# openGemini/openGemini

Measured on AMD Instinct MI355X. Metric: points aggregated/sec, higher is better.
Workload: dtype f64; 1 GPU; 100k series x 1k pts float64 Gorilla, mean/min/max/count GROUP BY time(1m), single TSSP file (mode=walk, 100000x1000); window=1m, series_per_gpu=100000, parallelism=shard-per-gpu dp1

## Files before the change

opengemini_amd/csrc/gemx_engine.hip:

```cpp
#include <hip/hip_runtime.h>
#include <stdint.h>
#include <stdio.h>
#include <string.h>
#include <stdlib.h>
#include <math.h>
#include <vector>
#include <map>
#include <tuple>
#include <type_traits>
#include <string>
#include <algorithm>
#include <chrono>

#include "../../include/gemx.h"

#define UVNAN 0x7FF8000000000001ULL
#define INFLUX_MIN_TIME (INT64_MIN + 2)
#define INFLUX_MAX_TIME (INT64_MAX - 1)


__device__ __forceinline__ uint32_t d_u32be(const uint8_t *p) {
  return ((uint32_t)p[0] << 24) | ((uint32_t)p[1] << 16) | ((uint32_t)p[2] << 8) |
         p[3];
}
// ... 23 lines not shown
  return b;
}
__device__ __forceinline__ int64_t d_zigzag_dec(uint64_t u) {
  return (int64_t)((u >> 1) ^ (uint64_t)((int64_t)((u & 1) << 63) >> 63));
}
__device__ __forceinline__ int d_uvarint(const uint8_t *p, int64_t len, uint64_t *out) {
  uint64_t v = 0;
  int s = 0;
  for (int i = 0; i < len && i < 10; i++) {
    uint8_t b = p[i];
    if (b < 0x80) {
      *out = v | ((uint64_t)b << s);
      return i + 1;
    }
    v |= (uint64_t)(b & 0x7f) << s;
    s += 7;
  }
  return 0;
}

__device__ __host__ __forceinline__ int64_t win_floordiv(int64_t a, int64_t b) {
  int64_t q = a / b;
  if ((a % b) != 0 && ((a < 0) != (b < 0))) q--;
  return q;
}
__device__ __host__ __forceinline__ int64_t win_ordinal(int64_t t, int64_t interval,
                                                        int64_t offset) {
  return win_floordiv(t - offset, interval);
}
__device__ __host__ __forceinline__ int64_t win_start_of(int64_t ord, int64_t interval,
                                                         int64_t offset) {
  int64_t s = ord * interval + offset;
  return s;
}


struct BitR {
  const uint8_t *b;
  int64_t len, pos;
  uint64_t hi, lo;
  int have;

  uint64_t pw;
  int pwbits;

  __device__ __forceinline__ void preload() {
    if (len - pos >= 8) {
      pw = d_u64be(b + pos);
      pos += 8;
      pwbits = 64;
    } else if (pos < len) {
      int rem = (int)(len - pos);
      uint64_t w = 0;
      for (int i = 0; i < rem; i++) w = (w << 8) | b[pos + i];
      pw = w << ((8 - rem) * 8);
      pos = len;
      pwbits = rem * 8;
    } else {
      pw = 0;
      pwbits = 0;
    }
  }

  __device__ __forceinline__ void fill_one() {
    unsigned __int128 ins = ((unsigned __int128)pw << 64) >> have;
    hi |= (uint64_t)(ins >> 64);
    lo |= (uint64_t)ins;
    have += pwbits;
    preload();
  }

  __device__ __forceinline__ void fill() {
    while (pwbits && have + pwbits <= 128) {
      if (have == 0) {
        hi = pw;
        lo = 0;
      } else if (have < 64) {
        hi |= pw >> have;
        lo |= pw << (64 - have);
      } else if (have == 64) {
        lo |= pw;
      } else {
        lo |= pw >> (have - 64);
      }
      have += pwbits;
      preload();
    }
  }

  __device__ __forceinline__ void init(const uint8_t *p, int64_t n) {
    b = p;
    len = n;
    pos = 0;
    hi = lo = 0;
    have = 0;
    pwbits = 0;
    preload();
    fill();
  }

  __device__ __forceinline__ int read(int n, uint64_t *out) {
    if (have < n) {
      fill();
      if (have < n) return -1;
    }
    uint64_t v = (n == 64) ? hi : (hi >> (64 - n));
    hi = (n == 64) ? lo : ((hi << n) | (lo >> (64 - n)));
    lo = (n == 64) ? 0 : (lo << n);
    have -= n;
    if (have <= 64) fill();
    *out = v;
    return 0;
  }

  __device__ __forceinline__ void consume(int n) {
    unsigned __int128 w = (((unsigned __int128)hi << 64) | lo) << n;
    hi = (uint64_t)(w >> 64);
    lo = (uint64_t)w;
    have -= n;
    if (have <= 64) fill_one();
  }
};

struct GorDesc {
  uint64_t first_val;
  uint64_t arena_base;
  int64_t t0, dt;
};

struct GorA {
  const uint64_t *p;
  uint64_t w0, w1, w2, w3;
  uint64_t M;
  uint32_t np;

  __device__ __forceinline__ void init(const uint64_t *arena, uint64_t base,
                                       uint32_t bp = 0) {
    p = arena + base;
    w0 = p[0 * 64];
    w1 = p[1 * 64];
    w2 = p[2 * 64];
    w3 = p[3 * 64];
    M = p[4 * 64];
    p += 4 * 64;
    np = bp;
  }
  __device__ __forceinline__ void advance(uint32_t nb) {
    np = nb;
    p += (uint64_t)(nb >> 6) << 6;
  }
  template <bool MASKED = true>
  __device__ __forceinline__ void settle() {
    const bool c = np >= 64;
    w0 = c ? w1 : w0;
    w1 = c ? w2 : w1;
    w2 = c ? w3 : w2;
    w3 = c ? M : w3;
    if (!MASKED || c) M = *p;
    if (__builtin_expect(__any(np >= 128), 0)) {
      const bool c2 = np >= 128;
      const uint64_t x = *(p - 64);
      asm volatile("" : "+v"(w1), "+v"(w2), "+v"(w3));
      w0 = c2 ? w1 : w0;
      w1 = c2 ? w2 : w1;
      w2 = c2 ? w3 : w2;
      w3 = c2 ? x : w3;
    }
    np &= 63;
  }
  __device__ __forceinline__ uint32_t word_idx(const uint64_t *base) const {
    return (uint32_t)((p - base) >> 6) - 4;
  }
  static __device__ __forceinline__ uint64_t fun(uint64_t a, uint64_t b,
                                                 uint32_t bp) {
    return (a << bp) | ((b >> (63 - bp)) >> 1);
  }
};

#define GEMX_ARENA_PAD_WORDS ((uint64_t)(2 * 4097 + 32) * 64)


struct FloatIter {
  int kind;
  const uint8_t *raw;
  int64_t raw_n, raw_i;
  double same_v;
  int64_t same_n, same_i;
  const uint8_t *rle_p;
  int64_t rle_len, rle_pos;
  int64_t run_left;
  double run_v;
  BitR br;
  GorA ga;
  int use_arena;
  uint64_t g_val;
  uint8_t g_trail, g_mean;
  int g_first, g_done;

  __device__ int init_gor_arena(const uint64_t *arena, const GorDesc *g) {
    kind = 3;
    use_arena = 1;
    g_val = g->first_val;
    g_done = (g_val == UVNAN);
    g_first = 1;
    g_trail = 0;
    g_mean = 64;
    ga.init(arena, g->arena_base);
    return 0;
  }

  __device__ int init(const uint8_t *enc, int64_t len) {
    if (len < 1) return -1;
    kind = enc[0] >> 4;
    const uint8_t *in = enc + 1;
    int64_t inlen = len - 1;
    switch (kind) {
    case 0:
      raw = in;
      raw_n = inlen / 8;
      raw_i = 0;
      return 0;
    case 4:
      if (inlen < 2) return -1;
      same_n = ((int64_t)in[0] << 8) | in[1];
      same_v = (inlen == 2) ? 0.0 : d_f64le(in + 2);
      same_i = 0;
      return 0;
    case 5:
      rle_p = in;
      rle_len = inlen;
      rle_pos = 0;
      run_left = 0;
      return 0;
    case 3:
      use_arena = 0;
      if (inlen < 9) { g_done = 1; g_first = 0; return 0; }
      g_val = d_u64be(in + 1);
      g_done = (g_val == UVNAN);
      g_first = 1;
      g_trail = 0;
      g_mean = 64;
      br.init(in + 9, inlen - 9);
      return 0;
    default:
      return -2;
    }
  }

  __device__ int next(double *out) {
    switch (kind) {
    case 0:
      if (raw_i >= raw_n) return -1;
      *out = d_f64le(raw + raw_i * 8);
      raw_i++;
      return 0;
    case 4:
      if (same_i >= same_n) return -1;
      *out = same_v;
      same_i++;
      return 0;
    case 5:
      while (run_left == 0) {
        if (rle_len - rle_pos < 2) return -1;
        uint16_t m = (uint16_t)(((uint16_t)rle_p[rle_pos] << 8) | rle_p[rle_pos + 1]);
        if (m >> 15) {
          run_left = m & 0x7FFF;
          run_v = 0.0;
          rle_pos += 2;
        } else {
          if (rle_len - rle_pos < 10) return -1;
          run_left = m;
          run_v = d_f64le(rle_p + rle_pos + 2);
          rle_pos += 10;
        }
      }
      *out = run_v;
      run_left--;
      return 0;
    case 3: {
      if (g_first) {
        if (g_done) return -1;
        g_first = 0;
        uint64_t u = g_val;
        memcpy(out, &u, 8);
        return 0;
      }
      if (g_done) return -1;
      if (use_arena) {
        uint64_t A = GorA::fun(ga.w0, ga.w1, ga.np);
        uint32_t p13 = (uint32_t)(A >> 51);
        uint32_t ctrl1 = p13 >> 12;
        uint32_t neww = ctrl1 & ((p13 >> 11) & 1);
        uint32_t mr = p13 & 0x3F;
        g_mean = neww ? (uint8_t)(mr ? mr : 64u) : g_mean;
        g_trail =
            neww ? (uint8_t)(mr ? (64u - ((p13 >> 6) & 0x1F) - mr) : 0u)
                 : g_trail;
        uint32_t hdr = 1 + ctrl1 + (neww ? 11u : 0u);
        uint64_t Cc = GorA::fun(ga.w1, ga.w2, ga.np);
        uint64_t B = (A << hdr) | (Cc >> (64 - hdr));
        uint64_t sbv = (g_mean == 64) ? B : (B >> (64 - g_mean));
        g_val ^= ctrl1 ? (sbv << (g_trail & 63)) : 0;
        if (g_val == UVNAN) {
          g_done = 1;
          return -1;
        }
        ga.advance(ga.np + hdr + (ctrl1 ? (uint32_t)g_mean : 0));
        ga.settle<false>();
        uint64_t u = g_val;
        memcpy(out, &u, 8);
        return 0;
// ... 1972 lines not shown
        at[op] = p.t[op];
        continue;
      }
      switch (op) {
      case 0: av[op].i += p.v[op].i; break;
      case 1:
        if (COLTYPE == GEMX_TYPE_FLOAT) av[op].f += p.v[op].f;
        else av[op].i += p.v[op].i;
        break;
      case 2: {
        int repl = (COLTYPE == GEMX_TYPE_FLOAT) ? (p.v[op].f < av[op].f)
                                                : (p.v[op].i < av[op].i);
        if (repl) { av[op] = p.v[op]; at[op] = p.t[op]; }
        break;
      }
      case 3: {
        int repl = (COLTYPE == GEMX_TYPE_FLOAT) ? (p.v[op].f > av[op].f)
                                                : (p.v[op].i > av[op].i);
        if (repl) { av[op] = p.v[op]; at[op] = p.t[op]; }
        break;
      }
      case 4: break;
      case 5: av[op] = p.v[op]; at[op] = p.t[op]; break;
      }
    }
  }
  if (!any) return 0;
  out->count = active[0] ? av[0].i : 0;
  out->count_time = active[0] ? at[0] : nt[0];
  out->sum = av[1];
  out->sum_time = active[1] ? at[1] : nt[1];
  out->sum_isnil = !active[1];
  out->minv = av[2];
  out->min_time = active[2] ? at[2] : nt[2];
  out->min_isnil = !active[2];
  out->maxv = av[3];
  out->max_time = active[3] ? at[3] : nt[3];
  out->max_isnil = !active[3];
  out->firstv = av[4];
  out->first_time = active[4] ? at[4] : nt[4];
  out->first_isnil = !active[4];
  out->lastv = av[5];
  out->last_time = active[5] ? at[5] : nt[5];
  out->last_isnil = !active[5];
  if (!active[1]) out->sum.i = 0;
  if (!active[2]) out->minv.i = 0;
  if (!active[3]) out->maxv.i = 0;
  if (!active[4]) out->firstv.i = 0;
  if (!active[5]) out->lastv.i = 0;
  return 1;
}

template <int COLTYPE>
__global__ void __launch_bounds__(256) k_merge(
    const SeriesQ *__restrict__ series, uint32_t nseries,
    const SegQ *__restrict__ segq, const Partial *__restrict__ partials,
    gemx_agg_row *__restrict__ rows, uint64_t total_rows, int64_t interval,
    int64_t offset, int64_t q_start, DevErr *__restrict__ err) {
  uint64_t gid = blockIdx.x * (uint64_t)blockDim.x + threadIdx.x;
  for (uint64_t r = gid; r < total_rows; r += gridDim.x * (uint64_t)blockDim.x) {
    uint32_t lo = 0, hi = nseries - 1;
    while (lo < hi) {
      uint32_t mid = (lo + hi + 1) >> 1;
      if (series[mid].out_base <= r) lo = mid;
      else hi = mid - 1;
    }
    const SeriesQ s = series[lo];
    int64_t w = s.w_min + (int64_t)(r - s.out_base);
    gemx_agg_row out;
    memset(&out, 0, sizeof(out));
    out.sid = s.sid;
    out.win_start = interval ? win_start_of(w, interval, offset) : q_start;
    if (!merge_series_window<COLTYPE>(s, segq, partials, w, &out)) {
      out.count = -1;
      __hip_atomic_fetch_add(&err->gaps, 1ull, __ATOMIC_RELAXED,
                            __HIP_MEMORY_SCOPE_SYSTEM);
    }
    rows[r] = out;
  }
}


template <int COLTYPE>
__device__ __forceinline__ void gacc_row(GAcc *a, const gemx_agg_row *r,
                                         uint32_t src) {
  a->used = 1;
  a->count += r->count;
  if (!r->sum_isnil) {
    if (!(a->active & 2)) {
      a->sum = r->sum;
      a->active |= 2;
    } else if (COLTYPE == GEMX_TYPE_FLOAT)
      a->sum.f += r->sum.f;
    else
      a->sum.i += r->sum.i;
  }
  if (!r->min_isnil) {
    int take = !(a->active & 4);
    if (!take) {
      take = (COLTYPE == GEMX_TYPE_FLOAT)
                 ? (r->minv.f < a->minv.f ||
                    (r->minv.f == a->minv.f && r->min_time < a->min_t))
                 : (r->minv.i < a->minv.i ||
                    (r->minv.i == a->minv.i && r->min_time < a->min_t));
    }
    if (take) {
      a->minv = r->minv;
      a->min_t = r->min_time;
      a->min_src = src;
      a->active |= 4;
    }
  }
  if (!r->max_isnil) {
    int take = !(a->active & 8);
    if (!take) {
      take = (COLTYPE == GEMX_TYPE_FLOAT)
                 ? (r->maxv.f > a->maxv.f ||
                    (r->maxv.f == a->maxv.f && r->max_time < a->max_t))
                 : (r->maxv.i > a->maxv.i ||
                    (r->maxv.i == a->maxv.i && r->max_time < a->max_t));
    }
    if (take) {
      a->maxv = r->maxv;
      a->max_t = r->max_time;
      a->max_src = src;
      a->active |= 8;
    }
  }
  if (!r->first_isnil) {
    if (!(a->active & 16) || r->first_time < a->first_t) {
      a->firstv = r->firstv;
      a->first_t = r->first_time;
      a->first_src = src;
      a->active |= 16;
    }
  }
  if (!r->last_isnil) {
    if (!(a->active & 32) || r->last_time > a->last_t) {
      a->lastv = r->lastv;
      a->last_t = r->last_time;
      a->last_src = src;
      a->active |= 32;
    }
  }
}

template <int COLTYPE>
__device__ __forceinline__ void gacc_merge(GAcc *l, const GAcc *r) {
  if (!r->used) return;
  l->used = 1;
  l->count += r->count;
  if (r->active & 2) {
    if (!(l->active & 2)) {
      l->sum = r->sum;
      l->active |= 2;
    } else if (COLTYPE == GEMX_TYPE_FLOAT)
      l->sum.f += r->sum.f;
    else
      l->sum.i += r->sum.i;
  }
  if (r->active & 4) {
    int take = !(l->active & 4);
    if (!take)
      take = (COLTYPE == GEMX_TYPE_FLOAT)
                 ? (r->minv.f < l->minv.f ||
                    (r->minv.f == l->minv.f &&
                     (r->min_t < l->min_t ||
                      (r->min_t == l->min_t && r->min_src < l->min_src))))
                 : (r->minv.i < l->minv.i ||
                    (r->minv.i == l->minv.i &&
                     (r->min_t < l->min_t ||
                      (r->min_t == l->min_t && r->min_src < l->min_src))));
    if (take) {
      l->minv = r->minv;
      l->min_t = r->min_t;
      l->min_src = r->min_src;
      l->active |= 4;
    }
  }
  if (r->active & 8) {
    int take = !(l->active & 8);
    if (!take)
      take = (COLTYPE == GEMX_TYPE_FLOAT)
                 ? (r->maxv.f > l->maxv.f ||
                    (r->maxv.f == l->maxv.f &&
                     (r->max_t < l->max_t ||
                      (r->max_t == l->max_t && r->max_src < l->max_src))))
                 : (r->maxv.i > l->maxv.i ||
                    (r->maxv.i == l->maxv.i &&
                     (r->max_t < l->max_t ||
                      (r->max_t == l->max_t && r->max_src < l->max_src))));
    if (take) {
      l->maxv = r->maxv;
      l->max_t = r->max_t;
      l->max_src = r->max_src;
      l->active |= 8;
    }
  }
  if (r->active & 16) {
    if (!(l->active & 16) || r->first_t < l->first_t ||
        (r->first_t == l->first_t && r->first_src < l->first_src)) {
      l->firstv = r->firstv;
      l->first_t = r->first_t;
      l->first_src = r->first_src;
      l->active |= 16;
    }
  }
  if (r->active & 32) {
    if (!(l->active & 32) || r->last_t > l->last_t ||
        (r->last_t == l->last_t && r->last_src < l->last_src)) {
      l->lastv = r->lastv;
      l->last_t = r->last_t;
      l->last_src = r->last_src;
      l->active |= 32;
    }
  }
}

template <int COLTYPE, bool FOLD = false>
__global__ void __launch_bounds__(256) k_group_p1(
    const SeriesQ *__restrict__ series, uint32_t nseries,
    const SegQ *__restrict__ segq, const Partial *__restrict__ partials,
    GAcc *__restrict__ gtmp, int64_t W0, uint32_t n_gwins, uint32_t split,
    uint32_t per_chunk, const uint32_t *__restrict__ sel = nullptr,
    const uint8_t *__restrict__ seg_folded = nullptr) {
  __shared__ GAcc sh[256];
  for (uint32_t bb = blockIdx.x; bb < n_gwins * split; bb += gridDim.x) {
    uint32_t wb = bb / split, c = bb % split;
    int64_t w = W0 + (int64_t)wb;
    uint32_t g0 = c * per_chunk;
    uint32_t g1 = g0 + per_chunk;
    if (g1 > nseries) g1 = nseries;
    GAcc a;
    memset(&a, 0, sizeof(a));
    for (uint32_t gi = g0 + threadIdx.x; gi < g1; gi += blockDim.x) {
      const uint32_t g = FOLD ? sel[gi] : gi;
      const SeriesQ s = series[g];
      int64_t local = w - s.w_min;
      if (local < 0 || local >= (int64_t)s.n_wins) continue;
      gemx_agg_row r;
      memset(&r, 0, sizeof(r));
      if (!merge_series_window<COLTYPE, FOLD>(s, segq, partials, w, &r,
                                              seg_folded))
        continue;
      gacc_row<COLTYPE>(&a, &r, g);
    }
    sh[threadIdx.x] = a;
    __syncthreads();
    for (int s2 = 128; s2 > 0; s2 >>= 1) {
      if (threadIdx.x < (uint32_t)s2)
        gacc_merge<COLTYPE>(&sh[threadIdx.x], &sh[threadIdx.x + s2]);
      __syncthreads();
    }
    if (threadIdx.x == 0) gtmp[bb] = sh[0];
    __syncthreads();
  }
}

template <int COLTYPE>
__global__ void __launch_bounds__(256) k_group_p2(
    const GAcc *__restrict__ gtmp, uint32_t split, gemx_agg_row *__restrict__ out,
    int64_t W0, uint32_t n_gwins, int64_t interval, int64_t offset,
    int64_t q_start, int keep_empty, DevErr *__restrict__ err,
    const GAcc *__restrict__ fold = nullptr, uint32_t n_fold = 0) {
  __shared__ GAcc sh[256];
  for (uint32_t wb = blockIdx.x; wb < n_gwins; wb += gridDim.x) {
    int64_t w = W0 + (int64_t)wb;
    GAcc a;
    memset(&a, 0, sizeof(a));
    for (uint32_t c = threadIdx.x; c < split; c += blockDim.x)
      gacc_merge<COLTYPE>(&a, &gtmp[wb * split + c]);
    for (uint32_t c = threadIdx.x; c < n_fold; c += blockDim.x)
      gacc_merge<COLTYPE>(&a, &fold[(uint64_t)wb * n_fold + c]);
    sh[threadIdx.x] = a;
    __syncthreads();
    for (int s = 128; s > 0; s >>= 1) {
      if (threadIdx.x < (uint32_t)s)
        gacc_merge<COLTYPE>(&sh[threadIdx.x], &sh[threadIdx.x + s]);
      __syncthreads();
    }
    if (threadIdx.x == 0) {
      GAcc *g = &sh[0];
      gemx_agg_row o;
      memset(&o, 0, sizeof(o));
      o.sid = 0;
      int64_t ws = interval ? win_start_of(w, interval, offset) : q_start;
      o.win_start = ws;
      if (!g->used) {
        if (keep_empty) {
          o.count = 0;
          o.first_row_time = ws;
          o.count_time = ws;
          o.sum_time = ws;
          o.min_isnil = o.max_isnil = o.first_isnil = o.last_isnil =
              o.sum_isnil = 1;
        } else {
          o.count = -1;
          __hip_atomic_fetch_add(&err->gaps, 1ull, __ATOMIC_RELAXED,
                            __HIP_MEMORY_SCOPE_SYSTEM);
        }
      } else {
        o.first_row_time = ws;
        o.count = g->count;
        o.count_time = ws;
        o.sum = g->sum;
        o.sum_time = ws;
        o.sum_isnil = !(g->active & 2);
        o.minv = g->minv;
        o.min_time = g->min_t;
        o.min_isnil = !(g->active & 4);
        o.maxv = g->maxv;
        o.max_time = g->max_t;
        o.max_isnil = !(g->active & 8);
        o.firstv = g->firstv;
        o.first_time = g->first_t;
        o.first_isnil = !(g->active & 16);
        o.lastv = g->lastv;
        o.last_time = g->last_t;
        o.last_isnil = !(g->active & 32);
      }
      out[wb] = o;
    }
    __syncthreads();
  }
}


template <int COLTYPE>
__global__ void __launch_bounds__(256) k_group_small(
    const SeriesQ *__restrict__ series, uint32_t nseries,
    const SegQ *__restrict__ segq, const Partial *__restrict__ partials,
    gemx_agg_row *__restrict__ out, int64_t W0, uint32_t n_gwins,
    int64_t interval, int64_t offset, int64_t q_start, int keep_empty,
    DevErr *__restrict__ err) {
  uint32_t gid = blockIdx.x * blockDim.x + threadIdx.x;
  for (uint32_t wb = gid; wb < n_gwins; wb += gridDim.x * blockDim.x) {
    int64_t w = W0 + (int64_t)wb;
    GAcc a;
    memset(&a, 0, sizeof(a));
    for (uint32_t g = 0; g < nseries; g++) {
      const SeriesQ sr = series[g];
      int64_t local = w - sr.w_min;
      if (local < 0 || local >= (int64_t)sr.n_wins) continue;
      gemx_agg_row r;
      memset(&r, 0, sizeof(r));
      if (!merge_series_window<COLTYPE>(sr, segq, partials, w, &r)) continue;
      gacc_row<COLTYPE>(&a, &r, g);
    }
    gemx_agg_row o;
    memset(&o, 0, sizeof(o));
    o.sid = 0;
    int64_t ws = interval ? win_start_of(w, interval, offset) : q_start;
    o.win_start = ws;
    if (!a.used) {
      if (keep_empty) {
        o.count = 0;
        o.first_row_time = ws;
        o.count_time = ws;
        o.sum_time = ws;
        o.min_isnil = o.max_isnil = o.first_isnil = o.last_isnil =
            o.sum_isnil = 1;
      } else {
        o.count = -1;
        __hip_atomic_fetch_add(&err->gaps, 1ull, __ATOMIC_RELAXED,
                               __HIP_MEMORY_SCOPE_SYSTEM);
      }
    } else {
      o.first_row_time = ws;
      o.count = a.count;
      o.count_time = ws;
      o.sum = a.sum;
      o.sum_time = ws;
      o.sum_isnil = !(a.active & 2);
      o.minv = a.minv;
      o.min_time = a.min_t;
      o.min_isnil = !(a.active & 4);
      o.maxv = a.maxv;
      o.max_time = a.max_t;
      o.max_isnil = !(a.active & 8);
      o.firstv = a.firstv;
      o.first_time = a.first_t;
      o.first_isnil = !(a.active & 16);
      o.lastv = a.lastv;
      o.last_time = a.last_t;
      o.last_isnil = !(a.active & 32);
    }
    out[wb] = o;
  }
}

struct TagChunk {
  uint32_t ser_off;
  uint32_t count;
  uint32_t off_in_grp;
  uint32_t _pad;
};

template <int COLTYPE>
__global__ void __launch_bounds__(256) k_tag_p1(
    const SeriesQ *__restrict__ series, const uint32_t *__restrict__ order,
    const TagChunk *__restrict__ chunks, uint32_t n_chunks,
    const SegQ *__restrict__ segq, const Partial *__restrict__ partials,
    GAcc *__restrict__ gtmp, int64_t W0, uint32_t n_gwins) {
  __shared__ GAcc sh[256];
  for (uint32_t bb = blockIdx.x; bb < n_gwins * n_chunks; bb += gridDim.x) {
    uint32_t wb = bb / n_chunks, c = bb % n_chunks;
    int64_t w = W0 + (int64_t)wb;
    const TagChunk ch = chunks[c];
    GAcc a;
    memset(&a, 0, sizeof(a));
    for (uint32_t i = threadIdx.x; i < ch.count; i += blockDim.x) {
      const uint32_t g = order[ch.ser_off + i];
      const SeriesQ s = series[g];
      int64_t local = w - s.w_min;
      if (local < 0 || local >= (int64_t)s.n_wins) continue;
      gemx_agg_row r;
      memset(&r, 0, sizeof(r));
      if (!merge_series_window<COLTYPE>(s, segq, partials, w, &r)) continue;
      gacc_row<COLTYPE>(&a, &r, ch.off_in_grp + i);
    }
    sh[threadIdx.x] = a;
    __syncthreads();
    for (int s2 = 128; s2 > 0; s2 >>= 1) {
      if (threadIdx.x < (uint32_t)s2)
        gacc_merge<COLTYPE>(&sh[threadIdx.x], &sh[threadIdx.x + s2]);
      __syncthreads();
    }
    if (threadIdx.x == 0) gtmp[bb] = sh[0];
    __syncthreads();
  }
}

template <int COLTYPE>
__global__ void __launch_bounds__(256) k_tag_p2(
    const GAcc *__restrict__ gtmp, const uint32_t *__restrict__ cstart,
    const uint32_t *__restrict__ ccount, uint32_t n_chunks,
    gemx_agg_row *__restrict__ out, uint32_t n_groups, int64_t W0,
    uint32_t n_gwins, int64_t interval, int64_t offset, int64_t q_start,
    DevErr *__restrict__ err) {
  uint64_t total = (uint64_t)n_groups * n_gwins;
  for (uint64_t r = blockIdx.x * (uint64_t)blockDim.x + threadIdx.x; r < total;
       r += gridDim.x * (uint64_t)blockDim.x) {
    uint32_t grp = (uint32_t)(r / n_gwins);
    uint32_t wb = (uint32_t)(r % n_gwins);
    int64_t w = W0 + (int64_t)wb;
    GAcc a;
    memset(&a, 0, sizeof(a));
    for (uint32_t j = 0; j < ccount[grp]; j++)
      gacc_merge<COLTYPE>(&a, &gtmp[(uint64_t)wb * n_chunks + cstart[grp] + j]);
    gemx_agg_row o;
    memset(&o, 0, sizeof(o));
    o.sid = grp;
    int64_t ws = interval ? win_start_of(w, interval, offset) : q_start;
    o.win_start = ws;
    if (!a.used) {
      o.count = -1;
      __hip_atomic_fetch_add(&err->gaps, 1ull, __ATOMIC_RELAXED,
                            __HIP_MEMORY_SCOPE_SYSTEM);
    } else {
      o.first_row_time = ws;
      o.count = a.count;
      o.count_time = ws;
      o.sum = a.sum;
      o.sum_time = ws;
      o.sum_isnil = !(a.active & 2);
      o.minv = a.minv;
      o.min_time = a.min_t;
      o.min_isnil = !(a.active & 4);
      o.maxv = a.maxv;
      o.max_time = a.max_t;
// ... 2584 lines not shown
      for (uint32_t i = 0; i < nser; i++) order[pos[T.group_ids[i]]++] = i;
      std::vector<TagChunk> chunks;
      std::vector<uint32_t> cstart(T.n_groups), ccount(T.n_groups);
      const uint32_t PER = 256;
      for (uint32_t g2 = 0; g2 < T.n_groups; g2++) {
        uint32_t a = gcnt[g2], b = gcnt[g2 + 1];
        cstart[g2] = (uint32_t)chunks.size();
        for (uint32_t o = a; o < b; o += PER)
          chunks.push_back({o, std::min(PER, b - o), o - a, 0});
        ccount[g2] = (uint32_t)chunks.size() - cstart[g2];
      }
      T.n_chunks = (uint32_t)chunks.size();
      if (T.n_chunks == 0) {
        chunks.push_back({0, 0, 0, 0});
      }
      HIP_CHECK(hipMalloc(&T.d_order, sizeof(uint32_t) * order.size()));
      HIP_CHECK(hipMemcpyAsync(T.d_order, order.data(),
                               sizeof(uint32_t) * order.size(),
                               hipMemcpyHostToDevice, s->stream));
      HIP_CHECK(hipMalloc(&T.d_chunks, sizeof(TagChunk) * chunks.size()));
      HIP_CHECK(hipMemcpyAsync(T.d_chunks, chunks.data(),
                               sizeof(TagChunk) * chunks.size(),
                               hipMemcpyHostToDevice, s->stream));
      HIP_CHECK(hipMalloc(&T.d_cstart,
                          sizeof(uint32_t) * (T.n_groups ? T.n_groups : 1)));
      HIP_CHECK(hipMalloc(&T.d_ccount,
                          sizeof(uint32_t) * (T.n_groups ? T.n_groups : 1)));
      if (T.n_groups) {
        HIP_CHECK(hipMemcpyAsync(T.d_cstart, cstart.data(),
                                 sizeof(uint32_t) * T.n_groups,
                                 hipMemcpyHostToDevice, s->stream));
        HIP_CHECK(hipMemcpyAsync(T.d_ccount, ccount.data(),
                                 sizeof(uint32_t) * T.n_groups,
                                 hipMemcpyHostToDevice, s->stream));
      }
      uint64_t gelems = (uint64_t)(P.n_gwins ? P.n_gwins : 1) *
                        (T.n_chunks ? T.n_chunks : 1);
      HIP_CHECK(hipMalloc(&T.d_gtmp, sizeof(GAcc) * gelems));
      uint64_t relems = (uint64_t)(T.n_groups ? T.n_groups : 1) *
                        (P.n_gwins ? P.n_gwins : 1);
      HIP_CHECK(hipMalloc(&T.d_rows, sizeof(gemx_agg_row) * relems));
      T.valid = true;
    }
    if (P.n_gwins > 0 && T.n_chunks > 0) {
      uint32_t b1 = (uint32_t)std::min<uint64_t>(
          (uint64_t)P.n_gwins * T.n_chunks, 65535);
      uint64_t total = (uint64_t)T.n_groups * P.n_gwins;
      uint32_t b2 =
          (uint32_t)std::min<uint64_t>((total + 255) / 256, 65535);
      if (s->col_type == GEMX_TYPE_FLOAT) {
        hipLaunchKernelGGL((k_tag_p1<GEMX_TYPE_FLOAT>), dim3(b1), dim3(256),
                           0, s->stream, d_sq, T.d_order, T.d_chunks,
                           T.n_chunks, d_segq, d_part, T.d_gtmp, P.W0,
                           (uint32_t)P.n_gwins);
        hipLaunchKernelGGL((k_tag_p2<GEMX_TYPE_FLOAT>), dim3(b2), dim3(256),
                           0, s->stream, (const GAcc *)T.d_gtmp, T.d_cstart,
                           T.d_ccount, T.n_chunks, T.d_rows, T.n_groups, P.W0,
                           (uint32_t)P.n_gwins, interval, offset, start_time,
                           d_err);
      } else {
        hipLaunchKernelGGL((k_tag_p1<GEMX_TYPE_INT>), dim3(b1), dim3(256), 0,
                           s->stream, d_sq, T.d_order, T.d_chunks, T.n_chunks,
                           d_segq, d_part, T.d_gtmp, P.W0,
                           (uint32_t)P.n_gwins);
        hipLaunchKernelGGL((k_tag_p2<GEMX_TYPE_INT>), dim3(b2), dim3(256), 0,
                           s->stream, (const GAcc *)T.d_gtmp, T.d_cstart,
                           T.d_ccount, T.n_chunks, T.d_rows, T.n_groups, P.W0,
                           (uint32_t)P.n_gwins, interval, offset, start_time,
                           d_err);
      }
    }
  }
  if (!tagq && !group_all && total_rows > 0) {
    uint32_t blocks = (uint32_t)std::min<uint64_t>((total_rows + TPB - 1) / TPB, 65535);
    if (s->col_type == GEMX_TYPE_FLOAT)
      hipLaunchKernelGGL((k_merge<GEMX_TYPE_FLOAT>), dim3(blocks), dim3(TPB), 0,
                         s->stream, d_sq, (uint32_t)sq.size(), d_segq, d_part, d_rows,
                         total_rows, interval, offset, start_time, d_err);
    else
      hipLaunchKernelGGL((k_merge<GEMX_TYPE_INT>), dim3(blocks), dim3(TPB), 0,
                         s->stream, d_sq, (uint32_t)sq.size(), d_segq, d_part, d_rows,
                         total_rows, interval, offset, start_time, d_err);
  }
  if (!tagq && group_all && P.n_gwins > 0 && sq.size() <= 32) {
    uint32_t bs = (uint32_t)std::min<uint64_t>((P.n_gwins + TPB - 1) / TPB,
                                               65535);
    if (s->col_type == GEMX_TYPE_FLOAT)
      hipLaunchKernelGGL((k_group_small<GEMX_TYPE_FLOAT>), dim3(bs),
                         dim3(TPB), 0, s->stream, d_sq, (uint32_t)sq.size(),
                         d_segq, d_part, P.d_grows2[slot], P.W0,
                         (uint32_t)P.n_gwins, interval, offset, start_time,
                         keep_empty, d_err);
    else
      hipLaunchKernelGGL((k_group_small<GEMX_TYPE_INT>), dim3(bs), dim3(TPB),
                         0, s->stream, d_sq, (uint32_t)sq.size(), d_segq,
                         d_part, P.d_grows2[slot], P.W0, (uint32_t)P.n_gwins,
                         interval, offset, start_time, keep_empty, d_err);
  } else if (!tagq && group_all && P.n_gwins > 0 && fold) {
    uint32_t b1 = (uint32_t)std::min<uint64_t>(P.n_gwins * P.fsplit, 65535);
    uint32_t b2 = (uint32_t)std::min<uint64_t>(P.n_gwins, 65535);
    if (P.n_p1_sel)
      hipLaunchKernelGGL((k_group_p1<GEMX_TYPE_FLOAT, true>), dim3(b1),
                         dim3(256), 0, s->stream, d_sq, P.n_p1_sel, d_segq,
                         d_part, (GAcc *)P.d_gtmp, P.W0, (uint32_t)P.n_gwins,
                         P.fsplit, P.fper_chunk, P.d_p1_sel, P.d_seg_folded);
    hipLaunchKernelGGL((k_group_p2<GEMX_TYPE_FLOAT>), dim3(b2), dim3(256), 0,
                       s->stream, (const GAcc *)P.d_gtmp,
                       P.n_p1_sel ? P.fsplit : 0u, P.d_grows2[slot], P.W0,
                       (uint32_t)P.n_gwins, interval, offset, start_time,
                       keep_empty, d_err, (const GAcc *)P.d_fold,
                       P.n_fold_waves);
  } else if (!tagq && group_all && P.n_gwins > 0) {
    uint32_t b1 = (uint32_t)std::min<uint64_t>(P.n_gwins * P.gsplit, 65535);
    uint32_t b2 = (uint32_t)std::min<uint64_t>(P.n_gwins, 65535);
    if (s->col_type == GEMX_TYPE_FLOAT) {
      hipLaunchKernelGGL((k_group_p1<GEMX_TYPE_FLOAT>), dim3(b1), dim3(256), 0,
                         s->stream, d_sq, (uint32_t)sq.size(), d_segq, d_part,
                         (GAcc *)P.d_gtmp, P.W0, (uint32_t)P.n_gwins, P.gsplit,
                         P.gper_chunk);
      hipLaunchKernelGGL((k_group_p2<GEMX_TYPE_FLOAT>), dim3(b2), dim3(256), 0,
                         s->stream, (const GAcc *)P.d_gtmp, P.gsplit,
                         P.d_grows2[slot], P.W0, (uint32_t)P.n_gwins, interval,
                         offset, start_time, keep_empty, d_err);
    } else {
      hipLaunchKernelGGL((k_group_p1<GEMX_TYPE_INT>), dim3(b1), dim3(256), 0,
                         s->stream, d_sq, (uint32_t)sq.size(), d_segq, d_part,
                         (GAcc *)P.d_gtmp, P.W0, (uint32_t)P.n_gwins, P.gsplit,
                         P.gper_chunk);
      hipLaunchKernelGGL((k_group_p2<GEMX_TYPE_INT>), dim3(b2), dim3(256), 0,
                         s->stream, (const GAcc *)P.d_gtmp, P.gsplit,
                         P.d_grows2[slot], P.W0, (uint32_t)P.n_gwins, interval,
                         offset, start_time, keep_empty, d_err);
    }
  }
  if (is_bool) {
    gemx_agg_row *er =
        tagq ? s->tag_plan.d_rows : (group_all ? P.d_grows2[slot] : d_rows);
    const uint64_t en = tagq ? (uint64_t)s->tag_plan.n_groups * P.n_gwins
                             : (group_all ? P.n_gwins : total_rows);
    if (en) {
      uint32_t bb = (uint32_t)std::min<uint64_t>((en + 255) / 256, 65535);
      hipLaunchKernelGGL(k_blank_sum, dim3(bb), dim3(256), 0, s->stream, er,
                         en);
    }
  }
  HIP_CHECK(hipEventRecord(ev2, s->stream));

  uint64_t fetch_rows = tagq ? (uint64_t)s->tag_plan.n_groups * P.n_gwins
                             : (group_all ? P.n_gwins : total_rows);
  if (fetch_rows > cap) {
    seterr("output capacity too small");
    return GEMX_E_CAP;
  }
  HIP_CHECK(hipStreamWaitEvent(s->copy_stream, ev2, 0));
  HIP_CHECK(hipMemcpyAsync(s->h_err2[slot], d_err, sizeof(DevErr),
                           hipMemcpyDeviceToHost, s->copy_stream));
  HIP_CHECK(hipMemcpyAsync(
      out_host,
      tagq ? s->tag_plan.d_rows : (group_all ? P.d_grows2[slot] : d_rows),
      sizeof(gemx_agg_row) * fetch_rows, hipMemcpyDeviceToHost,
      s->copy_stream));
  HIP_CHECK(hipEventRecord(s->ev_copy[slot], s->copy_stream));

  if (async_begin) {
    auto &pe = s->pend[(s->pend_head + s->pend_count) & 1];
    pe.active = true;
    pe.slot = slot;
    pe.fetch_rows = fetch_rows;
    pe.out = out_host;
    s->pend_count++;
    if (n_out) *n_out = 0;
    return GEMX_OK;
  }
  return scan_deliver(s, slot, fetch_rows, out_host, n_out, stats);
}

static int scan_deliver(gemx_shard *s, int slot, uint64_t fetch_rows,
                        gemx_agg_row *out_host, uint64_t *n_out,
                        gemx_query_stats *stats) {
  auto t_sync0 = std::chrono::steady_clock::now();
  HIP_CHECK(hipEventSynchronize(s->ev_copy[slot]));
  auto t_sync1 = std::chrono::steady_clock::now();

  float ms_scan = 0, ms_merge = 0, ms_total = 0;
  (void)hipEventElapsedTime(&ms_scan, s->ev_q[slot][0], s->ev_q[slot][1]);
  (void)hipEventElapsedTime(&ms_merge, s->ev_q[slot][1], s->ev_q[slot][2]);
  (void)hipEventElapsedTime(&ms_total, s->ev_q[slot][0], s->ev_q[slot][2]);

  const DevErr herr = *s->h_err2[slot];
  if (herr.code != 0) {
    seterr(herr.code == GEMX_E_UNSUPPORTED ? "unsupported codec on device"
                                           : "segment decode failed on device");
    return herr.code;
  }
  if (s->fold_q[slot].folded && herr.fold_nan != 0) {
    QueryPlan &P = s->plan;
    s->fold_q[slot].folded = false;
    P.fold_off = true;
    return scan_impl(s, P.start, P.end, P.interval, P.offset, 1, 0, 0, 0,
                     out_host, s->fold_q[slot].cap, n_out, stats, nullptr,
                     nullptr, 0, nullptr, nullptr, s->fold_q[slot].keep_empty,
                     slot);
  }

  uint64_t n = 0;
  if (herr.gaps == 0) {
    n = fetch_rows;
  } else {
    uint64_t i = 0;
    while (i < fetch_rows && out_host[i].count >= 0) i++;
    n = i;
    for (; i < fetch_rows; i++) {
      if (out_host[i].count < 0) continue;
      out_host[n] = out_host[i];
      n++;
    }
  }
  *n_out = n;
  auto t_comp = std::chrono::steady_clock::now();
  double sync_ms = std::chrono::duration<double, std::milli>(t_sync1 - t_sync0).count();
  double comp_ms = std::chrono::duration<double, std::milli>(t_comp - t_sync1).count();

  if (stats) {
    stats->decode_ms = ms_scan;
    stats->merge_ms = ms_merge;
    stats->total_ms = ms_total;
    stats->points = s->total_rows_scanned;
    stats->compressed_bytes = s->total_compressed_bytes;
    stats->n_rows = n;
    stats->h2d_ms = sync_ms + comp_ms;
  }
  return GEMX_OK;
}

extern "C" int gemx_fold_stats(gemx_shard *s, uint64_t *folded_segments,
                               uint64_t *scanned_segments, uint32_t *redone) {
  if (!s) return GEMX_E_INVALID;
  if (folded_segments) *folded_segments = s->last_fold_folded;
  if (scanned_segments) *scanned_segments = s->last_fold_scanned;
  if (redone) *redone = s->last_fold_redo;
  return GEMX_OK;
}

extern "C" int gemx_fold_split_stats(gemx_shard *s, uint32_t *k_max,
                                     uint32_t *tasks, uint64_t *skipped_rows) {
  if (!s) return GEMX_E_INVALID;
  if (k_max) *k_max = s->last_split_kmax;
  if (tasks) *tasks = s->last_split_tasks;
  if (skipped_rows) *skipped_rows = s->last_split_skipped;
  return GEMX_OK;
}

extern "C" int gemx_bool_stats(gemx_shard *s, uint64_t *bitpar_segments,
                               uint64_t *other_segments) {
  if (!s) return GEMX_E_INVALID;
  if (bitpar_segments) *bitpar_segments = s->last_bool_bitpar;
  if (other_segments) *other_segments = s->last_bool_other;
  return GEMX_OK;
}

extern "C" int gemx_scan_agg(gemx_shard *s, int64_t start_time, int64_t end_time,
                             int64_t interval, int64_t offset,
                             gemx_agg_row *out_host, uint64_t cap, uint64_t *n_out,
                             gemx_query_stats *stats) {
  return scan_impl(s, start_time, end_time, interval, offset, 0, 0, 0, 0,
                   out_host, cap, n_out, stats);
}

extern "C" int gemx_scan_agg_grouped(gemx_shard *s, int64_t start_time,
                                     int64_t end_time, int64_t interval,
                                     int64_t offset, gemx_agg_row *out_host,
                                     uint64_t cap, uint64_t *n_out,
                                     gemx_query_stats *stats) {
  return scan_impl(s, start_time, end_time, interval, offset, 1, 0, 0, 0,
                   out_host, cap, n_out, stats);
}

static int prom_rate_impl(gemx_shard *s, int64_t start_time, int64_t end_time,
                          int64_t range_ns, int64_t step_ns, int is_rate,
                          int is_counter, int func, gemx_rate_row *out_host,
                          uint64_t cap, uint64_t *n_out,
                          gemx_query_stats *stats, int async_begin = 0,
                          double scalar = 0.0, double scalar2 = 0.0) {
  if (!s) return GEMX_E_INVALID;
  if (async_begin && func >= GEMX_PF_QUANTILE) {
    seterr("quantile/mad are synchronous (host prefix-sum phase)");
    return GEMX_E_INVALID;
  }
  if (async_begin && s->rpend_count >= 2) {
    seterr("two rate queries already in flight: call gemx_prom_finish");
    return GEMX_E_INVALID;
  }
  if (!async_begin && s->rpend_count > 0) {
    seterr("async rate queries in flight: call gemx_prom_finish first");
    return GEMX_E_INVALID;
  }
  if (s->col_type != GEMX_TYPE_FLOAT) {
    seterr("prom rate needs a float column");
    return GEMX_E_INVALID;
  }
  if (range_ns <= 0 || step_ns < 0) {
    seterr("invalid range/step");
    return GEMX_E_INVALID;
  }
  if (step_ns > 0 && range_ns / step_ns + 2 > RATE_W) {
    seterr("range/step+2 exceeds the open-window ring (8) — unsupported this round");
    return GEMX_E_UNSUPPORTED;
  }
  HIP_CHECK(hipSetDevice(s->device));
  const uint64_t nsegs = s->nsegs;
  const uint64_t scratch_per_lane = seg_scratch_bytes(SEG_SPARE_PAGE);

  int64_t start_sample = start_time + range_ns;
  if (end_time < start_sample) {
    *n_out = 0;
// ... 1036 lines not shown
```

Baseline: 343.7 billion points/s.

## Rework bit-reader settle, group reduction with wave shuffles, and sync fetch stream

Replaces the select-based register shift in the Gorilla bit-reader settle with a branch plus inline v_mov_b64 moves. The group pass-2 reduction now loads four entries per thread per step and finishes with a two-step shared-memory stage followed by wavefront shuffles, which cuts shared memory use and barrier count. Union copies are changed to integer-member copies. For synchronous queries, result copies are issued on the compute stream instead of a separate copy stream plus event wait. The inline asm and shuffle code add risk around register constraints and correctness.

```diff
diff --git a/opengemini_amd/csrc/gemx_engine.hip b/opengemini_amd/csrc/gemx_engine.hip
--- a/opengemini_amd/csrc/gemx_engine.hip
+++ b/opengemini_amd/csrc/gemx_engine.hip
@@ -199,11 +199,21 @@
   template <bool MASKED = true>
   __device__ __forceinline__ void settle() {
     const bool c = np >= 64;
-    w0 = c ? w1 : w0;
-    w1 = c ? w2 : w1;
-    w2 = c ? w3 : w2;
-    w3 = c ? M : w3;
-    if (!MASKED || c) M = *p;
+    if constexpr (MASKED) {
+      if (c) {
+        asm volatile("v_mov_b64 %0, %1\n\tv_mov_b64 %1, %2\n\t"
+                     "v_mov_b64 %2, %3\n\tv_mov_b64 %3, %4"
+                     : "+v"(w0), "+v"(w1), "+v"(w2), "+v"(w3)
+                     : "v"(M));
+        M = *p;
+      }
+    } else {
+      w0 = c ? w1 : w0;
+      w1 = c ? w2 : w1;
+      w2 = c ? w3 : w2;
+      w3 = c ? M : w3;
+      M = *p;
+    }
     if (__builtin_expect(__any(np >= 128), 0)) {
       const bool c2 = np >= 128;
       const uint64_t x = *(p - 64);
@@ -2482,7 +2492,7 @@
   l->count += r->count;
   if (r->active & 2) {
     if (!(l->active & 2)) {
-      l->sum = r->sum;
+      l->sum.i = r->sum.i;
       l->active |= 2;
     } else if (COLTYPE == GEMX_TYPE_FLOAT)
       l->sum.f += r->sum.f;
@@ -2502,7 +2512,7 @@
                      (r->min_t < l->min_t ||
                       (r->min_t == l->min_t && r->min_src < l->min_src))));
     if (take) {
-      l->minv = r->minv;
+      l->minv.i = r->minv.i;
       l->min_t = r->min_t;
       l->min_src = r->min_src;
       l->active |= 4;
@@ -2521,7 +2531,7 @@
                      (r->max_t < l->max_t ||
                       (r->max_t == l->max_t && r->max_src < l->max_src))));
     if (take) {
-      l->maxv = r->maxv;
+      l->maxv.i = r->maxv.i;
       l->max_t = r->max_t;
       l->max_src = r->max_src;
       l->active |= 8;
@@ -2530,7 +2540,7 @@
   if (r->active & 16) {
     if (!(l->active & 16) || r->first_t < l->first_t ||
         (r->first_t == l->first_t && r->first_src < l->first_src)) {
-      l->firstv = r->firstv;
+      l->firstv.i = r->firstv.i;
       l->first_t = r->first_t;
       l->first_src = r->first_src;
       l->active |= 16;
@@ -2539,7 +2549,7 @@
   if (r->active & 32) {
     if (!(l->active & 32) || r->last_t > l->last_t ||
         (r->last_t == l->last_t && r->last_src < l->last_src)) {
-      l->lastv = r->lastv;
+      l->lastv.i = r->lastv.i;
       l->last_t = r->last_t;
       l->last_src = r->last_src;
       l->active |= 32;
@@ -2588,29 +2598,79 @@
 }
 
 template <int COLTYPE>
+__device__ __forceinline__ void gacc_fold_entries(GAcc &a,
+                                                  const GAcc *__restrict__ e,
+                                                  uint32_t n) {
+  constexpr uint32_t B = 4;
+  for (uint32_t c = threadIdx.x; c < n; c += B * 256) {
+    GAcc r[B];
+#pragma unroll
+    for (uint32_t j = 0; j < B; j++) {
+      const uint32_t cj = c + j * 256;
+      r[j] = e[cj < n ? cj : n - 1];
+      if (cj >= n) r[j].used = 0;
+    }
+#pragma unroll
+    for (uint32_t j = 0; j < B; j++) gacc_merge<COLTYPE>(&a, &r[j]);
+  }
+}
+
+__device__ __forceinline__ int64_t d_shd_i64(int64_t v, int s) {
+  const uint32_t lo = (uint32_t)__shfl_down((int)(uint32_t)v, s, 64);
+  const uint32_t hi =
+      (uint32_t)__shfl_down((int)(uint32_t)((uint64_t)v >> 32), s, 64);
+  return (int64_t)(((uint64_t)hi << 32) | lo);
+}
+__device__ __forceinline__ GAcc gacc_shfl_down(const GAcc &a, int s) {
+  GAcc r;
+  r.count = d_shd_i64(a.count, s);
+  r.sum.i = d_shd_i64(a.sum.i, s);
+  r.minv.i = d_shd_i64(a.minv.i, s);
+  r.maxv.i = d_shd_i64(a.maxv.i, s);
+  r.firstv.i = d_shd_i64(a.firstv.i, s);
+  r.lastv.i = d_shd_i64(a.lastv.i, s);
+  r.min_t = d_shd_i64(a.min_t, s);
+  r.max_t = d_shd_i64(a.max_t, s);
+  r.first_t = d_shd_i64(a.first_t, s);
+  r.last_t = d_shd_i64(a.last_t, s);
+  r.min_src = (uint32_t)__shfl_down((int)a.min_src, s, 64);
+  r.max_src = (uint32_t)__shfl_down((int)a.max_src, s, 64);
+  r.first_src = (uint32_t)__shfl_down((int)a.first_src, s, 64);
+  r.last_src = (uint32_t)__shfl_down((int)a.last_src, s, 64);
+  r.active = (uint32_t)__shfl_down((int)a.active, s, 64);
+  r.used = (uint32_t)__shfl_down((int)a.used, s, 64);
+  return r;
+}
+
+template <int COLTYPE>
 __global__ void __launch_bounds__(256) k_group_p2(
     const GAcc *__restrict__ gtmp, uint32_t split, gemx_agg_row *__restrict__ out,
     int64_t W0, uint32_t n_gwins, int64_t interval, int64_t offset,
     int64_t q_start, int keep_empty, DevErr *__restrict__ err,
     const GAcc *__restrict__ fold = nullptr, uint32_t n_fold = 0) {
-  __shared__ GAcc sh[256];
+  __shared__ GAcc sh[128 + 64];
+  const uint32_t t = threadIdx.x;
   for (uint32_t wb = blockIdx.x; wb < n_gwins; wb += gridDim.x) {
     int64_t w = W0 + (int64_t)wb;
     GAcc a;
     memset(&a, 0, sizeof(a));
-    for (uint32_t c = threadIdx.x; c < split; c += blockDim.x)
-      gacc_merge<COLTYPE>(&a, &gtmp[wb * split + c]);
-    for (uint32_t c = threadIdx.x; c < n_fold; c += blockDim.x)
-      gacc_merge<COLTYPE>(&a, &fold[(uint64_t)wb * n_fold + c]);
-    sh[threadIdx.x] = a;
+    gacc_fold_entries<COLTYPE>(a, gtmp + (uint64_t)wb * split, split);
+    gacc_fold_entries<COLTYPE>(a, fold + (uint64_t)wb * n_fold, n_fold);
+    if (t >= 128) sh[t - 128] = a;
     __syncthreads();
-    for (int s = 128; s > 0; s >>= 1) {
-      if (threadIdx.x < (uint32_t)s)
-        gacc_merge<COLTYPE>(&sh[threadIdx.x], &sh[threadIdx.x + s]);
-      __syncthreads();
-    }
-    if (threadIdx.x == 0) {
-      GAcc *g = &sh[0];
+    if (t < 128) gacc_merge<COLTYPE>(&a, &sh[t]);
+    if (t >= 64 && t < 128) sh[128 + t - 64] = a;
+    __syncthreads();
+    if (t < 64) {
+      gacc_merge<COLTYPE>(&a, &sh[128 + t]);
+#pragma unroll
+      for (int s = 32; s > 0; s >>= 1) {
+        const GAcc r = gacc_shfl_down(a, s);
+        gacc_merge<COLTYPE>(&a, &r);
+      }
+    }
+    if (t == 0) {
+      const GAcc *g = &a;
       gemx_agg_row o;
       memset(&o, 0, sizeof(o));
       o.sid = 0;
@@ -2633,19 +2693,19 @@
         o.first_row_time = ws;
         o.count = g->count;
         o.count_time = ws;
-        o.sum = g->sum;
+        o.sum.i = g->sum.i;
         o.sum_time = ws;
         o.sum_isnil = !(g->active & 2);
-        o.minv = g->minv;
+        o.minv.i = g->minv.i;
         o.min_time = g->min_t;
         o.min_isnil = !(g->active & 4);
-        o.maxv = g->maxv;
+        o.maxv.i = g->maxv.i;
         o.max_time = g->max_t;
         o.max_isnil = !(g->active & 8);
-        o.firstv = g->firstv;
+        o.firstv.i = g->firstv.i;
         o.first_time = g->first_t;
         o.first_isnil = !(g->active & 16);
-        o.lastv = g->lastv;
+        o.lastv.i = g->lastv.i;
         o.last_time = g->last_t;
         o.last_isnil = !(g->active & 32);
       }
@@ -5536,15 +5596,16 @@
     seterr("output capacity too small");
     return GEMX_E_CAP;
   }
-  HIP_CHECK(hipStreamWaitEvent(s->copy_stream, ev2, 0));
+  hipStream_t fetch_stream = async_begin ? s->copy_stream : s->stream;
+  if (async_begin) HIP_CHECK(hipStreamWaitEvent(s->copy_stream, ev2, 0));
   HIP_CHECK(hipMemcpyAsync(s->h_err2[slot], d_err, sizeof(DevErr),
-                           hipMemcpyDeviceToHost, s->copy_stream));
+                           hipMemcpyDeviceToHost, fetch_stream));
   HIP_CHECK(hipMemcpyAsync(
       out_host,
       tagq ? s->tag_plan.d_rows : (group_all ? P.d_grows2[slot] : d_rows),
       sizeof(gemx_agg_row) * fetch_rows, hipMemcpyDeviceToHost,
-      s->copy_stream));
-  HIP_CHECK(hipEventRecord(s->ev_copy[slot], s->copy_stream));
+      fetch_stream));
+  HIP_CHECK(hipEventRecord(s->ev_copy[slot], fetch_stream));
 
   if (async_begin) {
     auto &pe = s->pend[(s->pend_head + s->pend_count) & 1];
```

Result: faster. 380.9 billion points/s, median of 6 (+10.8%).
